# SunYangtian/Splatter_A_Video

Hardware: AMD Instinct MI355X
Metric: rendered frames/sec fwd+bwd @480p, 300k Gaussians (higher is better)
Workload: dtype f32

## Files before the change

splatter_a_video_amd/csrc/blend.hip:

```cpp
#include <stdlib.h>

#include <utility>

#include "common.h"
#include "blend_power.h"

struct BlendArgs {
    int P, C;
    int c0, cn;
    const float2 *uv;
    const float *conic;
    const float *opacity;
    const float *feature;
    const float *bias;
    const int *idx_sorted;
    const int2 *tile_range;
    float bg;
    const float *bgc;
    int W, H, gx;
    int K, trunc;
    float *out;
    float *final_T;
    int *ncontrib;
    int *gs_idx;
// ... 1033 lines not shown
    static constexpr int NA = (CH + 15) / 16;
    static constexpr int NK = (CH + 3) / 4;
    static constexpr bool SHARED = CH > 20;
    static constexpr int NSLAB = SHARED ? 1 : 4;
};

#define SCAN4(op, sh)                                                     \
    op " %0, %0, %0 row_shr:" sh " row_mask:0xf bank_mask:0xf\n\t"        \
    op " %1, %1, %1 row_shr:" sh " row_mask:0xf bank_mask:0xf\n\t"        \
    op " %2, %2, %2 row_shr:" sh " row_mask:0xf bank_mask:0xf\n\t"        \
    op " %3, %3, %3 row_shr:" sh " row_mask:0xf bank_mask:0xf\n\t"
__device__ __forceinline__ void row_scan_mul4(float &a, float &b, float &c, float &d) {
    asm volatile("s_nop 1\n\t" SCAN4("v_mul_f32_dpp", "1") SCAN4("v_mul_f32_dpp", "2") SCAN4("v_mul_f32_dpp", "4")
                     SCAN4("v_mul_f32_dpp", "8")
                 : "+v"(a), "+v"(b), "+v"(c), "+v"(d));
}
__device__ __forceinline__ void row_scan_add4(float &a, float &b, float &c, float &d) {
    asm volatile("s_nop 1\n\t" SCAN4("v_add_f32_dpp", "1") SCAN4("v_add_f32_dpp", "2") SCAN4("v_add_f32_dpp", "4")
                     SCAN4("v_add_f32_dpp", "8")
                 : "+v"(a), "+v"(b), "+v"(c), "+v"(d));
}
__device__ __forceinline__ void lds_store2_lane15(float *p, float a, float b) {
    const unsigned addr = (unsigned)(size_t)p;
    asm volatile(
        "s_mov_b64 exec, %3\n\t"
        "ds_write2_b32 %0, %1, %2 offset1:1\n\t"
        "s_mov_b64 exec, -1"
        :
        : "v"(addr), "v"(a), "v"(b), "s"(0x8000800080008000ull)
        : "memory");
}

template <int O0, int O1, int O2, int O3>
__device__ __forceinline__ void lds_store2x4_lane15(float *base, float a0, float b0, float a1, float b1, float a2, float b2, float a3,
                                                    float b3) {
    static_assert(O0 >= 0 && O1 >= 0 && O2 >= 0 && O3 >= 0 && O0 < 255 && O1 < 255 && O2 < 255 && O3 < 255, "ds_write2_b32 offsets are 8-bit dword counts");
    const unsigned addr = (unsigned)(size_t)base;
    asm volatile(
        "s_mov_b64 exec, %9\n\t"
        "ds_write2_b32 %0, %1, %2 offset0:%c10 offset1:%c11\n\t"
        "ds_write2_b32 %0, %3, %4 offset0:%c12 offset1:%c13\n\t"
        "ds_write2_b32 %0, %5, %6 offset0:%c14 offset1:%c15\n\t"
        "ds_write2_b32 %0, %7, %8 offset0:%c16 offset1:%c17\n\t"
        "s_mov_b64 exec, -1"
        :
        : "v"(addr), "v"(a0), "v"(b0), "v"(a1), "v"(b1), "v"(a2), "v"(b2), "v"(a3), "v"(b3), "s"(0x8000800080008000ull), "n"(O0),
          "n"(O0 + 1), "n"(O1), "n"(O1 + 1), "n"(O2), "n"(O2 + 1), "n"(O3), "n"(O3 + 1)
        : "memory");
}

typedef unsigned u32x2_b __attribute__((ext_vector_type(2)));
__device__ __forceinline__ float rows_sum(float v, int lane) {
    (void)lane;
    {
        const u32x2_b r = __builtin_amdgcn_permlane16_swap(__float_as_uint(v), __float_as_uint(v), false, false);
        v = __uint_as_float(r[0]) + __uint_as_float(r[1]);
    }
    {
        const u32x2_b r = __builtin_amdgcn_permlane32_swap(__float_as_uint(v), __float_as_uint(v), false, false);
        v = __uint_as_float(r[0]) + __uint_as_float(r[1]);
    }
    return v;
}

__device__ __forceinline__ void row_shr1_add4(float (&R)[4], const float (&rs)[4], const float (&base)[4]) {
    asm volatile(
        "s_nop 1\n\t"
        "v_add_f32_dpp %0, %4, %8 row_shr:1 row_mask:0xf bank_mask:0xf bound_ctrl:1\n\t"
        "v_add_f32_dpp %1, %5, %9 row_shr:1 row_mask:0xf bank_mask:0xf bound_ctrl:1\n\t"
        "v_add_f32_dpp %2, %6, %10 row_shr:1 row_mask:0xf bank_mask:0xf bound_ctrl:1\n\t"
        "v_add_f32_dpp %3, %7, %11 row_shr:1 row_mask:0xf bank_mask:0xf bound_ctrl:1\n\t"
        : "=&v"(R[0]), "=&v"(R[1]), "=&v"(R[2]), "=&v"(R[3])
        : "v"(rs[0]), "v"(rs[1]), "v"(rs[2]), "v"(rs[3]), "v"(base[0]), "v"(base[1]), "v"(base[2]), "v"(base[3]));
}


template <int QP>
struct QuarterWalk {
    static constexpr float CEN = 0.5f * (float)(QP + 3);
    static __device__ __forceinline__ int qx(int q) { return QP * ((q >> 4) & 1) + (q & 3); }
    static __device__ __forceinline__ int qy(int q) { return QP * (q >> 5) + ((q >> 2) & 3); }
};

template <typename Walk>
__device__ __forceinline__ void strip_phi(int nl, int kk, float ox, float oy, float (&phi1)[4], float (&phi2)[4]) {
#pragma unroll
    for (int Gs = 0; Gs < 4; ++Gs) {
        const int q = 16 * Gs + nl;
        const float x = (float)Walk::qx(q) + ox, y = (float)Walk::qy(q) + oy;
        phi1[Gs] = kk == 0 ? 1.f : kk == 1 ? x : kk == 2 ? y : x * x;
        phi2[Gs] = kk == 0 ? x * y : kk == 1 ? y * y : 0.f;
    }
}

template <typename Walk>
__device__ __forceinline__ void strip_moment_table(float (&s_mom)[16 * 32], int w, int nl, int kk) {
#pragma unroll
    for (int r = 0; r < 4; ++r) {
        const int st = 4 * w + r, Gs = st >> 2, is = st & 3;
        const int q = 16 * Gs + 4 * kk + is;
        const float x = (float)Walk::qx(q) - Walk::CEN, y = (float)Walk::qy(q) - Walk::CEN;
        float v = 0.f;
        if (nl < 4) v = nl == 0 ? 1.f : nl == 1 ? x : nl == 2 ? y : x * x;
        else if (nl < 6) v = nl == 4 ? x * y : y * y;
        if (nl < 8) s_mom[32 * st + 8 * kk + nl] = v;
    }
}

template <int SB>
__device__ __forceinline__ unsigned load_flags(const unsigned int *cull_flags, int tid, int first, int topb) {
    const int q = topb - tid;
    return (tid < SB && q >= 0) ? (unsigned)cull_flags[first + q] : 0u;
}

template <int SB, bool TRANSPOSE, int NKEEP>
__device__ __forceinline__ void keep_from_quarter_flags(unsigned int (&s_keep)[NKEEP], const int (&s_wmax)[4], int tid, int nb, int top, unsigned fl) {
    static_assert(NKEEP >= SB, "a keep word per staged entry");
    if (tid < SB) {
        unsigned kw = 0u;
        if (tid < nb) {
#pragma unroll
            for (int ww = 0; ww < 4; ++ww) {
                if (TRANSPOSE) {
                    const unsigned t4 = (fl >> ww) & 0x01010101u;
                    const unsigned nib = ((t4 * 0x01020408u) >> 24) & 0xfu;
                    if (top - tid < s_wmax[ww]) kw |= nib << (8 * ww);
                } else {
                    if (top - tid < s_wmax[ww]) kw |= fl & (0xfu << (8 * ww));
                }
            }
        }
        s_keep[tid] = kw;
    }
}

__device__ __forceinline__ unsigned wave_scan_bytes4(unsigned word) {
    unsigned incl = word;
    asm volatile("s_nop 1\n\t"
                 "v_add_u32_dpp %0, %0, %0 row_shr:1 row_mask:0xf bank_mask:0xf\n\t"
                 "s_nop 1\n\t"
                 "v_add_u32_dpp %0, %0, %0 row_shr:2 row_mask:0xf bank_mask:0xf\n\t"
                 "s_nop 1\n\t"
                 "v_add_u32_dpp %0, %0, %0 row_shr:4 row_mask:0xf bank_mask:0xf\n\t"
                 "s_nop 1\n\t"
                 "v_add_u32_dpp %0, %0, %0 row_shr:8 row_mask:0xf bank_mask:0xf\n\t"
                 "s_nop 1\n\t"
                 "v_add_u32_dpp %0, %0, %0 row_bcast:15 row_mask:0xa bank_mask:0xf\n\t"
                 "s_nop 1\n\t"
                 "v_add_u32_dpp %0, %0, %0 row_bcast:31 row_mask:0xc bank_mask:0xf\n\t"
                 : "+v"(incl));
    return incl;
}

template <int SB, int CAP, int RW, bool ROUNDS, int NKEEP, typename List>
__device__ __forceinline__ int build_quarter_lists(const unsigned int (&s_keep)[NKEEP], unsigned int (&s_pos4)[NKEEP], List list, float *slab,
                                                   int w, int lane, int (&cq)[4], int p0 = 0, int *more = nullptr) {
    static_assert(ROUNDS || CAP >= SB, "one round: a slab row per staged entry");
    static_assert(NKEEP >= (SB + WAVE - 1) / WAVE * WAVE, "every lane of a pass reads a keep word");
    unsigned cqw = 0u;
    int cnt = 0;
#pragma unroll
    for (int r = 0; r < (SB + WAVE - 1) / WAVE; ++r) {
        const int e = r * WAVE + lane;
        unsigned bits = (s_keep[e] >> (8 * w)) & 0xfu;
        const bool kb = bits != 0u;
        const unsigned long long m = __builtin_amdgcn_ballot_w64(kb);
        const int ps = cnt + __builtin_amdgcn_mbcnt_hi((unsigned)(m >> 32), __builtin_amdgcn_mbcnt_lo((unsigned)m, 0u));
        if (!ROUNDS) reinterpret_cast<unsigned char *>(s_pos4)[4 * e + w] = kb ? (unsigned char)ps : (unsigned char)255;
        else if (p0 == 0) reinterpret_cast<unsigned char *>(s_pos4)[4 * e + w] = kb ? (unsigned char)imin_(ps, 254) : (unsigned char)255;
        if (ROUNDS) bits = ((unsigned)(ps - p0) < (unsigned)CAP) ? bits : 0u;
        const unsigned word = (bits * 0x00204081u) & 0x01010101u;
        const unsigned incl = wave_scan_bytes4(word);
        const unsigned posw = cqw + incl - word;
        const unsigned short ent = (unsigned short)(e | ((ROUNDS ? ps - p0 : ps) << 8));
#pragma unroll
        for (int q = 0; q < 4; ++q)
            if ((bits >> q) & 1u) list(q, (posw >> (8 * q)) & 0xffu) = ent;
        cqw += (unsigned)__builtin_amdgcn_readlane((int)incl, 63);
        cnt += __popcll(m);
    }
#pragma unroll
    for (int q = 0; q < 4; ++q) cq[q] = (int)((cqw >> (8 * q)) & 0xffu);
    if (lane < 16) {
#pragma unroll
        for (int q = 0; q < 4; ++q) list(q, cq[q] + lane) = (unsigned short)(SB | (CAP << 8));
    }
    {
        const int rows = ROUNDS ? imin_(imax_(cnt - p0, 0), CAP) : cnt;
        float4 *z = reinterpret_cast<float4 *>(slab);
        for (int c = lane; c < rows * (RW / 4); c += WAVE) z[c] = make_float4(0.f, 0.f, 0.f, 0.f);
    }
    if (ROUNDS && lane == 0) *more = cnt > p0 + CAP;
    __builtin_amdgcn_fence(__ATOMIC_RELEASE, "wavefront");
    __builtin_amdgcn_wave_barrier();
    return cnt;
}

template <int NSEC, int LAST, int RS>
struct QuadStager {
    int id_next;
    float4 v[NSEC];

    __device__ __forceinline__ QuadStager() {
        if (LAST < 4) v[NSEC - 1] = make_float4(0.f, 0.f, 0.f, 0.f);
    }
    template <typename Pos>
    __device__ __forceinline__ void load_ids(const BlendArgs &A, int tid, int base, Pos pos, int batch) {
        const int q = pos(tid >> 2, batch);
        id_next = q >= 0 ? A.idx_sorted[base + q] : -1;
    }
    __device__ __forceinline__ void load_payload(const BlendArgs &A, int tid) {
        const int sp = tid & 3;
        const float4 *src = reinterpret_cast<const float4 *>(A.pack + (size_t)imax_(id_next, 0) * RS) + sp;
#pragma unroll
        for (int k = 0; k < NSEC - 1; ++k) v[k] = src[4 * k];
        if (LAST == 4 || (LAST > 0 && sp < LAST)) v[NSEC - 1] = src[4 * (NSEC - 1)];
    }
};

__device__ __forceinline__ void pair_exchange_geometry(const float4 &mine, bool first, float4 &g0, float4 &g1) {
    float4 other;
    other.x = __int_as_float(__builtin_amdgcn_mov_dpp(__float_as_int(mine.x), 0xB1, 0xf, 0xf, true));
    other.y = __int_as_float(__builtin_amdgcn_mov_dpp(__float_as_int(mine.y), 0xB1, 0xf, 0xf, true));
    other.z = __int_as_float(__builtin_amdgcn_mov_dpp(__float_as_int(mine.z), 0xB1, 0xf, 0xf, true));
    other.w = __int_as_float(__builtin_amdgcn_mov_dpp(__float_as_int(mine.w), 0xB1, 0xf, 0xf, true));
    g0 = first ? mine : other;
    g1 = first ? other : mine;
}

__device__ __forceinline__ void store_T_front(const BlendArgs &A, int px, int py, const float &t) {
    if (A.dbg_T_front) {
        if (px < A.W && py < A.H) A.dbg_T_front[(size_t)A.W * py + px] = t;
    }
}

template <int CH, int NK, int NA>
__device__ __forceinline__ void hoist_dl_dout(float *stage, const float (&gpix)[CH], int lane, float (&hcg)[4][NK], float (&hft)[16][NA]) {
    const int nl = lane & 15, kk = lane >> 4;
#pragma unroll
    for (int h = 0; h < 2; ++h) {
        if ((lane >> 5) == h) {
#pragma unroll
            for (int k = 0; k < CH; ++k) stage[(lane & 31) * CH + k] = gpix[k];
        }
        __builtin_amdgcn_fence(__ATOMIC_RELEASE, "wavefront");
        __builtin_amdgcn_wave_barrier();
#pragma unroll
        for (int G = 2 * h; G < 2 * h + 2; ++G)
#pragma unroll
            for (int j = 0; j < NK; ++j) hcg[G][j] = stage[(16 * (G & 1) + nl) * CH + 4 * j + kk];
#pragma unroll
        for (int st = 8 * h; st < 8 * h + 8; ++st) {
#pragma unroll
            for (int q = 0; q < NA; ++q)
                hft[st][q] = 16 * q + nl < CH ? stage[(16 * ((st >> 2) & 1) + 4 * kk + (st & 3)) * CH + 16 * q + nl] : 0.f;
        }
        __builtin_amdgcn_fence(__ATOMIC_ACQUIRE, "wavefront");
        __builtin_amdgcn_wave_barrier();
    }
}

template <int CH, bool ABS, bool EXACT>
__global__ void __launch_bounds__(256, (MfmaCfg<CH, ABS>::MINW))
blend_bwd_mfma_kernel(const BlendArgs B) {
    using Cfg = MfmaCfg<CH, ABS>;
    constexpr int SB = Cfg::SB, NG = Cfg::NG, NC = Cfg::NC, NCP = Cfg::NCP, PW = Cfg::PW, NA = Cfg::NA, NK = Cfg::NK;
    constexpr int PZ = Cfg::PZ, PS = Cfg::PS;
    constexpr int I_ABS = GradLayout<ABS, false>::I_ABS;
    constexpr bool SHARED = Cfg::SHARED;
    constexpr bool CARRY = CH <= 20;
    constexpr int CQ = CarryLDS<SB>::CQ, XR = CARRY ? 4 * CQ : 0;
    constexpr int CAP = SHARED ? (1 << 20) : (!CARRY ? SB : ((SB == 128 && NC <= 9) ? 80 : 64));
    constexpr int TPR = (NC + 2) / 3, NCS = SHARED ? 3 * TPR : NC;
    constexpr int SROWS = SHARED ? SB + XR : CAP + (CARRY ? 1 : 0);
    __shared__ TileLDS<CH, SB, false, XR, true> L;
    __shared__ CarryLDS<SB, !SHARED> CL;
    constexpr bool FEAT_VALU = CH <= 4;
    __shared__ float s_acc[Cfg::NSLAB][SROWS * NCS];
    constexpr int KS = 4 * PW + 8, GS = 4 * KS;
    __shared__ __attribute__((aligned(16))) float s_pix[4][4 * GS];
    auto pixoff = [](int q) { return (q >> 4) * GS + ((q >> 2) & 3) * KS + (q & 3) * PW; };
    __shared__ float s_mom[16 * 64];
    __shared__ int s_wmax[4];
    const int tid = threadIdx.x, lane = tid & 63, w = tid >> 6;
    const int gtile = xcd_tile(blockIdx.x, gridDim.x);
    const int frame = gtile / B.T, tile = gtile - frame * B.T;
    const BlendArgs A = frame_args(B, frame);
    const int RST = B.rec_stride ? B.rec_stride : NCP;
    float *const pair_buf = B.pair_buf + (size_t)frame * (size_t)B.cap * RST + B.rec_off;
    const int tx = tile % A.gx, ty = tile / A.gx;
    const int bx = tx * TILE + (w & 1) * 8, by = ty * TILE + (w >> 1) * 8;
    const float bx0 = (float)bx, by0 = (float)by;
    const float tcx = (float)(tx * TILE) + 7.5f, tcy = (float)(ty * TILE) + 7.5f;
    const float ox = (float)((w & 1) * 8) - 7.5f, oy = (float)((w >> 1) * 8) - 7.5f;
    const int cn = EXACT ? CH : A.cn;
    const int nl = lane & 15, kk = lane >> 4;
    int wmax;
#pragma unroll
    for (int r = 0; r < 4; ++r) {
        const int st = 4 * w + r, Gs = st >> 2, is = st & 3;
        const int q = 16 * Gs + 4 * kk + is;
        const float x = (float)(q & 7) - 3.5f, y = (float)(q >> 3) - 3.5f;
        const int grp = nl >> 2, i = nl & 3;
        float v = 0.f;
        if (grp == 0) v = i == 0 ? 1.f : i == 1 ? x : i == 2 ? y : x * x;
        if (grp == 1) v = i == 0 ? 1.f : i == 1 ? x : i == 2 ? y : x * y;
        if (grp == 2) v = i == 0 ? 1.f : i == 1 ? y : i == 2 ? y * y : 0.f;
        s_mom[64 * st + lane] = v;
    }
    float phi1[4], phi2[4];
#pragma unroll
    for (int Gs = 0; Gs < 4; ++Gs) {
        const int q = 16 * Gs + nl;
        const float x = (float)(q & 7) + ox, y = (float)(q >> 3) + oy;
        phi1[Gs] = kk == 0 ? 1.f : kk == 1 ? x : kk == 2 ? y : x * x;
        phi2[Gs] = kk == 0 ? x * y : kk == 1 ? y * y : 0.f;
    }
    {
        const int px = bx + (lane & 7), py = by + (lane >> 3);
        const size_t HW = (size_t)A.H * A.W;
        const bool inside = (px < A.W) && (py < A.H);
        const size_t pix = (size_t)A.W * (size_t)py + px;
        const float Tf = inside ? A.final_T[pix] : 0.f;
        const int last = inside ? A.ncontrib[pix] : 0;
        float *r = s_pix[w] + pixoff(lane);
        float bgdot = 0.f;
#pragma unroll
        for (int k = 0; k < CH; ++k) {
            const float g = (inside && k < cn) ? A.dL_dout[(size_t)(A.c0 + k) * HW + pix] : 0.f;
            r[k] = g;
            bgdot += A.bg * g;
        }
#pragma unroll
        for (int k = CH; k < PS; ++k) r[k] = 0.f;
        r[PS] = 0.f;
        r[PS + 1] = __int_as_float(last);
        r[PS + 2] = Tf;
        r[PS + 3] = Tf * bgdot;
// ... 209 lines not shown
            }
            if (j0 + nl < nproc) {
                float *rec = slab + (SHARED ? (e > SB ? e - 1 : e) : (CARRY ? j0 + nl - p0 : e)) * NCS;
                auto put = [](float *p, float v) {
                    if (SHARED) __hip_atomic_fetch_add(p, v, __ATOMIC_RELAXED, __HIP_MEMORY_SCOPE_WORKGROUP);
                    else *p = v;
                };
                const float D0 = d_mom[0];
                if (kk == 0) {
                    const float Dx = d_mom[1], Dy = d_mom[2], Dxx = d_mom[3];
                    put(rec + 0, cA * Dx + cB * Dy - (cA * uc + cB * vc) * D0);
                    put(rec + 1, cB * Dx + cC * Dy - (cB * uc + cC * vc) * D0);
                    put(rec + 2, -0.5f * (uc * uc * D0 - 2.f * uc * Dx + Dxx));
                    put(rec + 5, o > 0.f ? D0 / o : 0.f);
                    if (ABS) {
                        put(rec + I_ABS, s_ax);
                        put(rec + I_ABS + 1, s_ay);
                    }
                } else if (kk == 1) {
                    const float Dx = d_mom[1], Dy = d_mom[2], Dxy = d_mom[3];
                    put(rec + 3, -(uc * vc * D0 - uc * Dy - vc * Dx + Dxy));
                } else if (kk == 2) {
                    const float Dy = d_mom[1], Dyy = d_mom[2];
                    put(rec + 4, -0.5f * (vc * vc * D0 - 2.f * vc * Dy + Dyy));
                }
                if (FEAT_VALU) {
                    if (kk == 3) {
#pragma unroll
                        for (int c = 0; c < (FEAT_VALU ? CH : 1); ++c) put(rec + NG + c, dfv[c]);
                    }
                } else {
#pragma unroll
                    for (int q = 0; q < NA; ++q)
#pragma unroll
                        for (int i = 0; i < 4; ++i) {
                            const int c = 16 * q + 4 * kk + i;
                            if (c < CH) put(rec + NG + c, d_f[q][i]);
                        }
                }
            }
        }
        if (CARRY && p0 == 0) {
            __builtin_amdgcn_fence(__ATOMIC_RELEASE, "wavefront");
            __builtin_amdgcn_wave_barrier();
            if (nproc > 0)
                for (int idx = lane; idx < ncin * NC; idx += 64) {
                    const int k = idx / NC, c = idx - k * NC;
                    float *src = SHARED ? slab + (SB + CQ * w + k) * NCS + c : slab + idx;
                    __hip_atomic_fetch_add(pair_buf + (size_t)CL.cslot[w][k] * RST + c, *src, __ATOMIC_RELAXED,
                                           __HIP_MEMORY_SCOPE_AGENT);
                    if (SHARED) *src = 0.f;
                }
            const int left = total - nproc;
            if (left > 0) carry_out<CH, SB>(L, CL, w, lane, nproc > 0 ? nproc : ncin, nproc > 0 ? left : left - ncin,
                                            nproc > 0 ? 0 : ncin, top, slots);
            ncarry = left;
        }
        if (CARRY && !SHARED && lane == 0) CL.more[w] = nproc > p0 + CAP;
        if (p0 == 0) {
            load_slots();
            st.load_payload(A, tid);
            st.load_ids(A, tid, range.x, pos, batch + 2);
        }
        __syncthreads();
        if (ce < EPI) {
            const int lo = top - nb + 1;
            if (SHARED) {
#pragma unroll
                for (int r = 0; r < NPASS; ++r) {
                    const int ql = ce + r * EPI;
                    if (ql < nb) {
                        float *row = s_acc[0] + (nb - 1 - ql) * NCS + CW * cc;
                        const float v0 = row[0], v1 = row[CW > 1 ? 1 : 0], v2 = row[CW > 1 ? 2 : 0];
                        row[0] = 0.f;
                        if (CW > 1) { row[1] = 0.f; row[2] = 0.f; }
                        store_part(NPASS <= 3 ? sl[NPASS <= 3 ? r : 0] : slots[lo + ql], v0, v1, v2);
                    }
                }
            } else {
#pragma unroll
                for (int r = 0; r < NPASS; ++r) {
                    const int ql = ce + r * EPI;
                    if (ql < nb) {
                        const unsigned int p4 = CL.pos4[nb - 1 - ql];
                        float v[3] = {0.f, 0.f, 0.f};
#pragma unroll
                        for (int ww = 0; ww < 4; ++ww) {
                            const unsigned int pp = umin_(((p4 >> (8 * ww)) & 0xffu) - (unsigned)p0, (unsigned)CAP);
                            const float *row = s_acc[ww] + pp * NC + CW * cc;
#pragma unroll
                            for (int j = 0; j < 3; ++j)
                                if (CW * (TPR - 1) + j < NC || CW * cc + j < NC) v[j] += row[j];
                        }
                        const int slot = NPASS <= 3 ? sl[NPASS <= 3 ? r : 0] : slots[lo + ql];
                        if (p0 > 0) {
                            const float *old = pair_buf + (size_t)slot * RST + CW * cc;
#pragma unroll
                            for (int j = 0; j < 3; ++j)
                                if (CW * cc + j < NCP) v[j] += old[j];
                        }
                        store_part(slot, v[0], v[1], v[2]);
                    }
                }
            }
        }
        if (SHARED) break;
        const bool more = CARRY && (CL.more[0] | CL.more[1] | CL.more[2] | CL.more[3]);
        __syncthreads();
        if (!more) break;
        }
    }
    if (A.dbg_T_front) {
        const int px = bx + (lane & 7), py = by + (lane >> 3);
        if (px < A.W && py < A.H) A.dbg_T_front[(size_t)A.W * py + px] = s_pix[w][pixoff(lane) + PS + 2];
    }
}

#define ROW_LANES(X) X(0) X(1) X(2) X(3) X(4) X(5) X(6) X(7) X(8) X(9) X(10) X(11) X(12) X(13) X(14) X(15)
__device__ __forceinline__ void fmac_row_lane(int n, float &acc, float src, float w) {
    switch (n) {
#define ROW_CASE(N) case N: asm("v_fmac_f32_dpp %0, %1, %2 row_newbcast:" #N " row_mask:0xf bank_mask:0xf" : "+v"(acc) : "v"(src), "v"(w)); break;
        ROW_LANES(ROW_CASE)
#undef ROW_CASE
    }
}
__device__ __forceinline__ void mul_row_lane(int n, float &acc, float src, float w) {
    switch (n) {
#define ROW_CASE(N) case N: asm("v_mul_f32_dpp %0, %1, %2 row_newbcast:" #N " row_mask:0xf bank_mask:0xf" : "=&v"(acc) : "v"(src), "v"(w)); break;
        ROW_LANES(ROW_CASE)
#undef ROW_CASE
    }
}
__device__ __forceinline__ int row_lane(int n, int v) {
    switch (n) {
#define ROW_CASE(N) case N: return __builtin_amdgcn_update_dpp(0, v, 0x150 + N, 0xf, 0xf, true);
        ROW_LANES(ROW_CASE)
#undef ROW_CASE
    }
    return v;
}
#undef ROW_LANES

template <int CH, bool ABS = false>
struct QuarterCfg {
    static_assert(CH <= 3 && Rec<CH>::RQ == 4 && Rec<CH>::CULL >= 11, "floats 11-15 of the record (cull parameters) are free for the coefficients");
    static constexpr int SB = 128;
    static constexpr int CAP = 80;
    static constexpr int MINW = ABS ? 3 : 4;
    static constexpr int NG = GradLayout<ABS, false>::NG, NC = NG + CH, NCP = PAIR_STRIDE(NC);
    static constexpr int RW = ABS ? 16 : 12;
    static constexpr int PW = 8;
};

template <int CH, bool ABS, bool EXACT>
__global__ void __launch_bounds__(256, (QuarterCfg<CH, ABS>::MINW))
blend_bwd_quarter_kernel(const BlendArgs B) {
    using Cfg = QuarterCfg<CH, ABS>;
    constexpr int SB = Cfg::SB, CAP = Cfg::CAP, NCP = Cfg::NCP, RW = Cfg::RW, PW = Cfg::PW, RQ = 4;
    static_assert(SB <= 128 && CAP < 255, "list entries are (entry | position << 8) in 16 bits");
    __shared__ float4 s_rec[(SB + 1) * RQ];
    auto qpart = [](int e, int p) { return 4 * e + (p ^ ((e >> 2) & 3)); };
    __shared__ unsigned int s_keep[SB];
    __shared__ unsigned short s_qlist[4][4][CAP + 16];
    __shared__ unsigned int s_pos4[SB];
    __shared__ __attribute__((aligned(16))) float s_acc[4][(CAP + 1) * RW];
    constexpr int KS = 4 * PW + 8, GS = 4 * KS;
    __shared__ __attribute__((aligned(16))) float s_pix[4][4 * GS];
    auto pixoff = [](int q) { return (q >> 4) * GS + ((q >> 2) & 3) * KS + (q & 3) * PW; };
    __shared__ float s_mom[16 * 32];
    __shared__ int s_wmax[4];
    __shared__ int s_more[4];
    const int tid = threadIdx.x, lane = tid & 63, w = tid >> 6;
    const int gtile = xcd_tile(blockIdx.x, gridDim.x);
    const int frame = gtile / B.T, tile = gtile - frame * B.T;
    const BlendArgs A = frame_args(B, frame);
    const int RST = B.rec_stride ? B.rec_stride : NCP;
    float *const pair_buf = B.pair_buf + (size_t)frame * (size_t)B.cap * RST + B.rec_off;
    const int tx = tile % A.gx, ty = tile / A.gx;
    const int bx = tx * TILE + (w & 1) * 8, by = ty * TILE + (w >> 1) * 8;
    const float tcx = (float)(tx * TILE) + 7.5f, tcy = (float)(ty * TILE) + 7.5f;
    const float ox = (float)((w & 1) * 8) - 7.5f, oy = (float)((w >> 1) * 8) - 7.5f;
    const int cn = EXACT ? CH : A.cn;
    const int nl = lane & 15, kk = lane >> 4;
    using Walk = QuarterWalk<4>;
#pragma unroll
    for (int r = 0; r < 4; ++r) {
        const int st = 4 * w + r, Gs = st >> 2, is = st & 3;
        const int q = 16 * Gs + 4 * kk + is;
        const float x = (float)Walk::qx(q) - Walk::CEN, y = (float)Walk::qy(q) - Walk::CEN;
        float v = 0.f;
        if (ABS) {
            if (nl < 4) v = nl == 0 ? 1.f : nl == 1 ? x : nl == 2 ? y : x * x;
            else if (nl < 6) v = nl == 4 ? x * y : y * y;
        } else {
            if (nl < 3) v = nl == 0 ? 1.f : nl == 1 ? x : y;
            else if (nl >= 4 && nl < 7) v = nl == 4 ? x * x : nl == 5 ? x * y : y * y;
        }
        if (nl < 8) s_mom[32 * st + 8 * kk + nl] = v;
    }
    float phi1[4], phi2[4];
    strip_phi<Walk>(nl, kk, ox, oy, phi1, phi2);
    const int lx = lane & 7, ly = lane >> 3;
    const int myq = 16 * ((lx >> 2) + 2 * (ly >> 2)) + 4 * (ly & 3) + (lx & 3);
    {
        const int px = bx + lx, py = by + ly;
        const size_t HW = (size_t)A.H * A.W;
        const bool inside = (px < A.W) && (py < A.H);
        const size_t pix = (size_t)A.W * (size_t)py + px;
        const float Tf = inside ? A.final_T[pix] : 0.f;
        const int last = inside ? A.ncontrib[pix] : 0;
        float *r = s_pix[w] + pixoff(myq);
        float bgdot = 0.f;
#pragma unroll
        for (int k = 0; k < 4; ++k) {
            const float g = (k < CH && inside && k < cn) ? A.dL_dout[(size_t)(A.c0 + k) * HW + pix] : 0.f;
            r[k] = g;
            bgdot += A.bg * g;
        }
        r[4] = 0.f;
        r[5] = __int_as_float(last);
        r[6] = Tf;
        r[7] = Tf * bgdot;
        const int wmax = wave_max_i(last);
        if (lane == 0) s_wmax[w] = wmax;
    }
    if (tid < RQ) s_rec[qpart(SB, tid)] = make_float4(tid == 3 ? -__builtin_inff() : 0.f, 0.f, 0.f, 0.f);
    if (lane < RW) s_acc[w][CAP * RW + lane] = 0.f;
    __syncthreads();
    const int2 range = A.tile_range[tile];
    const int len = range.y - range.x;
    const int n = imin_(len, imax_(imax_(s_wmax[0], s_wmax[1]), imax_(s_wmax[2], s_wmax[3])));
    const int *slots = A.slot_sorted + range.x;
    auto store_rec = [&](int slot, const float (&v)[12]) {
        float4 *dst = reinterpret_cast<float4 *>(pair_buf + (size_t)slot * RST);
#pragma unroll
        for (int c = 0; c < NCP / 4; ++c) dst[c] = make_float4(v[4 * c], v[4 * c + 1], v[4 * c + 2], v[4 * c + 3]);
    };
    {
        const float z[12] = {0.f, 0.f, 0.f, 0.f, 0.f, 0.f, 0.f, 0.f, 0.f, 0.f, 0.f, 0.f};
        for (int ql = n + tid; ql < len; ql += 256) store_rec(slots[ql], z);
    }
    if (n <= 0) {
        store_T_front(A, bx + lx, by + ly, s_pix[w][pixoff(myq) + 6]);
        return;
    }
    float *pixrow = s_pix[w] + kk * KS;
    float gpix[3];
    int lastpix;
    {
        const float *r = s_pix[w] + (nl >> 2) * GS + kk * KS + (nl & 3) * PW;
        gpix[0] = r[0]; gpix[1] = r[1]; gpix[2] = r[2];
        lastpix = __float_as_int(r[5]);
    }
    const float *pixcol = s_pix[w] + pixoff(nl);
    const float *momrow = s_mom + 8 * kk + (nl & 7);
    const int kch = kk < CH ? kk : 4;

    auto pos = [n](int e, int b) { return n - 1 - b * SB - e; };
    Stager<CH, SB> st;
    static_assert(Stager<CH, SB>::NCHUNK % 256 == 0, "every thread parks K chunks");
    st.load_ids(A, tid, range.x, pos, 0);
    st.load_payload(A, tid);
    st.load_ids(A, tid, range.x, pos, 1);
    unsigned fl_next = load_flags<SB>(A.cull_flags, tid, range.x, n - 1);

    int batch = 0;
    for (int top = n - 1; top >= 0; top -= SB, ++batch) {
        const int nb = imin_(SB, top + 1);
        {
            const int p = tid & 3;
#pragma unroll
            for (int k = 0; k < Stager<CH, SB>::K; ++k) {
                const int e = (tid >> 2) + 64 * k;
                const float4 mine = st.v[k];
                float4 g0, g1;
                pair_exchange_geometry(mine, p == 0, g0, g1);
                const PowerCoef pc = power_coeffs(g0.x, g0.y, g0.z, g0.w, g1.x, g1.y, tcx, tcy);
                if (p == 0) {
                    s_rec[qpart(e, 0)] = mine;
                    s_rec[qpart(e, 3)] = make_float4(pc.q0, pc.qx, pc.qy, pc.qxx);
                } else if (p == 1) {
                    s_rec[qpart(e, 1)] = make_float4(mine.x, mine.y, pc.qxy, pc.qyy);
                } else if (p == 2) {
                    s_rec[qpart(e, 2)] = make_float4(mine.x, mine.y, mine.z, 0.f);
                }
            }
        }
        const unsigned fl = fl_next;
        fl_next = load_flags<SB>(A.cull_flags, tid, range.x, top - SB);
        keep_from_quarter_flags<SB, false>(s_keep, s_wmax, tid, nb, top, fl);
        __syncthreads();
        float *slab = s_acc[w];
        int slot_mine = 0;
        for (int p0 = 0;; p0 += CAP) {
            int cq[4];
            build_quarter_lists<SB, CAP, RW, true>(s_keep, s_pos4, [&](int q, int i) -> unsigned short & { return s_qlist[w][q][i]; }, slab, w, lane, cq, p0,
                                                   &s_more[w]);
#pragma unroll
            for (int G = 0; G < 4; ++G) {
                const float cgA = pixcol[G * GS + kch];
                float momA[4];
#pragma unroll
                for (int i = 0; i < 4; ++i) momA[i] = momrow[32 * (4 * G + i)];
                for (int j0 = 0; j0 < cq[G]; j0 += 16) {
                    const unsigned le = s_qlist[w][G][j0 + nl];
                    const int e = le & 0xffu, row = le >> 8;
                    const int qn = top - e;
                    const float *er = reinterpret_cast<const float *>(s_rec) + e * (4 * RQ);
                    const int sw = 4 * ((e >> 2) & 3);
                    const float bq1 = er[(12 ^ sw) + kk];
                    const float bq2 = er[(4 ^ sw) + 2 + (kk & 1)];
                    const float bf = er[(8 ^ sw) + kk];
                    float blx = 0.f, bly = 0.f;
                    if (ABS) {
                        const float4 ge = *reinterpret_cast<const float4 *>(er + (0 ^ sw));
                        const float cCe = er[(4 ^ sw)];
                        const float ut = ge.x - tcx, vt = ge.y - tcy;
                        blx = kk == 0 ? -(ge.z * ut + ge.w * vt) : kk == 1 ? ge.z : kk == 2 ? ge.w : 0.f;
                        bly = kk == 0 ? -(ge.w * ut + cCe * vt) : kk == 1 ? ge.w : kk == 2 ? cCe : 0.f;
                    }
                    float s_ax = 0.f, s_ay = 0.f;
                    f32x4 d_mom = {0.f, 0.f, 0.f, 0.f};
                    float dfv[CH];
                    asm volatile("" ::: "memory");
                    f32x4 pw = {0.f, 0.f, 0.f, 0.f}, cgv = {0.f, 0.f, 0.f, 0.f};
                    pw = __builtin_amdgcn_mfma_f32_16x16x4f32(phi1[G], bq1, pw, 0, 0, 0);
                    pw = __builtin_amdgcn_mfma_f32_16x16x4f32(phi2[G], bq2, pw, 0, 0, 0);
                    cgv = __builtin_amdgcn_mfma_f32_16x16x4f32(cgA, bf, cgv, 0, 0, 0);
                    float cg[4], araw[4], a[4], r1a[4], rp[4], Ts4[4], Rs4[4];
#pragma unroll
                    for (int i = 0; i < 4; ++i) {
                        const float2 stv = *reinterpret_cast<const float2 *>(pixrow + G * GS + i * PW + 6);
                        cg[i] = cgv[i];
                        const int last = row_lane(4 * G + i, lastpix);
                        Ts4[i] = stv.x;
                        Rs4[i] = stv.y;
                        bool pw_ok;
                        araw[i] = exp2_guard(pw[i], pw_ok);
                        const bool ok = (qn < last) && pw_ok && !(araw[i] < (1.0f / 255.0f));
                        araw[i] = ok ? araw[i] : 0.f;
                        a[i] = fminf(0.99f, araw[i]);
                        r1a[i] = __builtin_amdgcn_rcpf(1.f - a[i]);
                        rp[i] = r1a[i];
                    }
                    row_scan_mul4(rp[0], rp[1], rp[2], rp[3]);
                    float T[4], wgt[4], rs[4], R[4];
#pragma unroll
                    for (int i = 0; i < 4; ++i) {
                        T[i] = Ts4[i] * rp[i];
                        wgt[i] = a[i] * T[i];
                        rs[i] = cg[i] * wgt[i];
                    }
                    row_scan_add4(rs[0], rs[1], rs[2], rs[3]);
                    row_shr1_add4(R, rs, Rs4);
                    lds_store2x4_lane15<6, PW + 6, 2 * PW + 6, 3 * PW + 6>(pixrow + G * GS, T[0], Rs4[0] + rs[0], T[1], Rs4[1] + rs[1], T[2],
                                                                           Rs4[2] + rs[2], T[3], Rs4[3] + rs[3]);
                    f32x4 lx4 = {0.f, 0.f, 0.f, 0.f}, ly4 = {0.f, 0.f, 0.f, 0.f};
                    if (ABS) {
                        lx4 = __builtin_amdgcn_mfma_f32_16x16x4f32(phi1[G], blx, lx4, 0, 0, 0);
                        ly4 = __builtin_amdgcn_mfma_f32_16x16x4f32(phi1[G], bly, ly4, 0, 0, 0);
                    }
#pragma unroll
                    for (int i = 0; i < 4; ++i) {
                        const float dLa = T[i] * cg[i] - R[i] * r1a[i];
                        const float dLp = araw[i] * dLa;
                        d_mom = __builtin_amdgcn_mfma_f32_16x16x4f32(momA[i], dLp, d_mom, 0, 0, 0);
                        if (ABS) {
                            s_ax += fabsf(dLp * lx4[i]);
                            s_ay += fabsf(dLp * ly4[i]);
                        }
#pragma unroll
                        for (int c = 0; c < CH; ++c) {
                            if (i == 0) mul_row_lane(4 * G, dfv[c], gpix[c], wgt[0]);
                            else fmac_row_lane(4 * G + i, dfv[c], gpix[c], wgt[i]);
                        }
                    }
                    if (ABS) {
                        s_ax = rows_sum(s_ax, lane);
                        s_ay = rows_sum(s_ay, lane);
                    }
                    float fs[3] = {0.f, 0.f, 0.f};
#pragma unroll
                    for (int c = 0; c < CH; ++c) {
                        const u32x2_b r = __builtin_amdgcn_permlane32_swap(__float_as_uint(dfv[c]), __float_as_uint(dfv[c]), false, false);
                        fs[c] = __uint_as_float(r[0]) + __uint_as_float(r[1]);
                    }
                    if (!ABS) {
                        if (j0 + nl < cq[G]) {
                            F3 *r3 = reinterpret_cast<F3 *>(slab + row * RW + 3 * kk);
                            F3 v3 = *r3;
                            v3.x += kk < 2 ? d_mom[0] : fs[0];
                            v3.y += kk < 2 ? d_mom[1] : fs[1];
                            v3.z += kk < 2 ? d_mom[2] : fs[2];
                            *r3 = v3;
                        }
                    } else if (kk < 2 && j0 + nl < cq[G]) {
                        float4 *rm = reinterpret_cast<float4 *>(slab + row * RW + 4 * kk), *rf = rm + 2;
                        float4 m4 = *rm, f4 = *rf;
                        m4.x += d_mom[0]; m4.y += d_mom[1];
                        m4.z += ABS ? d_mom[2] + (kk == 1 ? s_ax : 0.f) : d_mom[2];
                        m4.w += ABS ? d_mom[3] + (kk == 1 ? s_ay : 0.f) : d_mom[3];
                        f4.x += fs[0]; f4.y += fs[1]; f4.z += fs[2];
                        *rm = m4;
                        *rf = f4;
                    }
                    __builtin_amdgcn_fence(__ATOMIC_RELEASE, "wavefront");
                    __builtin_amdgcn_wave_barrier();
                }
            }
            if (p0 == 0) {
                slot_mine = tid < nb ? slots[top - tid] : 0;
                st.load_payload(A, tid);
                st.load_ids(A, tid, range.x, pos, batch + 2);
            }
            __syncthreads();
            if (tid < nb) {
                const int e = tid;
                const unsigned int p4 = s_pos4[e];
                float s[12] = {0.f, 0.f, 0.f, 0.f, 0.f, 0.f, 0.f, 0.f, 0.f, 0.f, 0.f, 0.f};
#pragma unroll
                for (int ww = 0; ww < 4; ++ww) {
                    const unsigned int pp = umin_(((p4 >> (8 * ww)) & 0xffu) - (unsigned)p0, (unsigned)CAP);
                    const float4 *rw = reinterpret_cast<const float4 *>(s_acc[ww] + pp * RW);
                    float4 m, m2, fa, fb;
                    if (ABS) {
                        m = rw[0]; m2 = rw[1]; fa = rw[2]; fb = rw[3];
                    } else {
                        const float4 r1 = rw[1], r2 = rw[2];
                        m = rw[0];
                        m2 = make_float4(r1.x, r1.y, 0.f, 0.f);
                        fa = make_float4(r1.z, r1.w, r2.x, 0.f);
                        fb = make_float4(r2.y, r2.z, r2.w, 0.f);
                    }
                    const float bxw = (ww & 1) ? 4.f : -4.f, byw = (ww >> 1) ? 4.f : -4.f;
                    s[0] += m.x;
                    s[1] += m.y + bxw * m.x;
                    s[2] += m.z + byw * m.x;
                    s[3] += m.w + 2.f * bxw * m.y + (bxw * bxw) * m.x;
                    s[4] += m2.x + bxw * m.z + byw * m.y + (bxw * byw) * m.x;
                    s[5] += m2.y + 2.f * byw * m.z + (byw * byw) * m.x;
                    s[6] += fa.x + fb.x; s[7] += fa.y + fb.y; s[8] += fa.z + fb.z;
                    s[9] += m2.z; s[10] += m2.w;
                }
                const float4 g0 = s_rec[qpart(e, 0)], g1 = s_rec[qpart(e, 1)];
                const float cA = g0.z, cB = g0.w, cC = g1.x, o = g1.y;
                const float uc = g0.x - tcx, vc = g0.y - tcy;
                const float M0 = s[0], Mx = s[1], My = s[2], Mxx = s[3], Mxy = s[4], Myy = s[5];
                float rec[12];
                rec[0] = cA * Mx + cB * My - (cA * uc + cB * vc) * M0;
                rec[1] = cB * Mx + cC * My - (cB * uc + cC * vc) * M0;
                rec[2] = -0.5f * (uc * uc * M0 - 2.f * uc * Mx + Mxx);
                rec[3] = -(uc * vc * M0 - uc * My - vc * Mx + Mxy);
                rec[4] = -0.5f * (vc * vc * M0 - 2.f * vc * My + Myy);
                rec[5] = o > 0.f ? M0 / o : 0.f;
                rec[6] = 0.f; rec[7] = 0.f; rec[8] = 0.f; rec[9] = 0.f; rec[10] = 0.f; rec[11] = 0.f;
                if (ABS) { rec[6] = s[9]; rec[7] = s[10]; }
                rec[Cfg::NG] = s[6];
                if (CH > 1) rec[Cfg::NG + 1 % CH] = s[7];
                if (CH > 2) rec[Cfg::NG + 2 % CH] = s[8];
                if (p0 > 0) {
                    const float *old = pair_buf + (size_t)slot_mine * RST;
#pragma unroll
                    for (int c = 0; c < Cfg::NC; ++c) rec[c] += old[c];
                }
                store_rec(slot_mine, rec);
            }
            const bool more = s_more[0] | s_more[1] | s_more[2] | s_more[3];
            __syncthreads();
            if (!more) break;
        }
    }
    store_T_front(A, bx + lx, by + ly, s_pix[w][pixoff(myq) + 6]);
}

struct SetsCfg {
    static constexpr int CH = 28, NK = 7, NA = 2, SB = 64;
    static constexpr int NG = SETS_NG, NCMAX = NG + CH;
    static constexpr int PS = 8;
    static constexpr int MINW = 2;
    static constexpr int CAP = 32;
};

__device__ __forceinline__ constexpr int sets_fpos(int slot) { return 8 + 8 * (slot & 3) + (slot >> 2); }

__device__ __forceinline__ int sets_slot_channel(const BlendArgs &A, int slot) {
    const int g = slot < 4 ? 0 : slot < 8 ? 1 : 2;
    const int o = slot - (g == 0 ? 0 : g == 1 ? 4 : 8);
    const int c0 = g == 0 ? A.s0c0 : g == 1 ? A.s1c0 : A.s2c0, cn = g == 0 ? A.s0cn : g == 1 ? A.s1cn : A.s2cn;
    return (slot < SetsCfg::CH && o < cn) ? c0 + o : -1;
}

__global__ void __launch_bounds__(256)
pack_sets_kernel(const BlendArgs B) {
    const BlendArgs A = frame_args(B, blockIdx.y);
    constexpr int CH = SetsCfg::CH, RS = Rec<CH>::RS, CO = Rec<CH>::CULL;
    static_assert(CO >= 0, "the cull parameters ride in the record's padding");
    constexpr int RQ = Rec<CH>::RQ, LS = RS + 4;
    __shared__ __attribute__((aligned(16))) float s_rec[256 * LS];
    const int i0 = blockIdx.x * 256;
    const int i = i0 + threadIdx.x;
    float r[RS];
#pragma unroll
    for (int k = 0; k < RS; ++k) r[k] = 0.f;
    if (i < A.P) {
        const float2 q = A.uv[i];
        r[0] = q.x; r[1] = q.y;
        r[2] = A.conic[3 * i]; r[3] = A.conic[3 * i + 1]; r[4] = A.conic[3 * i + 2];
        r[5] = A.opacity[i];
        r[7] = __int_as_float(i);
        if (A.feature) {
            const float *f = A.feature + (size_t)i * (A.feature_row ? A.feature_row : A.C);
#pragma unroll
            for (int k = 0; k < CH; ++k) {
                const int c = sets_slot_channel(A, k);
                if (c >= 0) r[sets_fpos(k)] = f[c];
            }
        }
        const CullP cp = cull_params(r[2], r[3], r[4], r[5]);
        r[CO] = cp.hx; r[CO + 1] = cp.hy; r[CO + 2] = cp.tauq; r[CO + 3] = cp.ia; r[CO + 4] = cp.ic;
    }
    float4 *row = reinterpret_cast<float4 *>(s_rec + threadIdx.x * LS);
#pragma unroll
    for (int k = 0; k < RS; k += 4) row[k / 4] = make_float4(r[k], r[k + 1], r[k + 2], r[k + 3]);
    __syncthreads();
    const int nrec = imin_(256, A.P - i0);
    if (!A.feature) {
        stage_feature_rows<true>(s_rec, LS, 0, A.sf0, A.s0cn, i0, nrec);
        stage_feature_rows<true>(s_rec, LS, 4, A.sf1, A.s1cn, i0, nrec);
        stage_feature_rows<true>(s_rec, LS, 8, A.sf2, A.s2cn, i0, nrec);
        __syncthreads();
    }
    float4 *dst = reinterpret_cast<float4 *>(A.pack + (size_t)i0 * RS);
    for (int c = threadIdx.x; c < nrec * RQ; c += 256) {
        const int g = c / RQ, part = c - g * RQ;
        dst[c] = *reinterpret_cast<const float4 *>(s_rec + g * LS + 4 * part);
    }
}

template <bool ABS>
__global__ void __launch_bounds__(256, SetsCfg::MINW)
blend_bwd_sets_kernel(const BlendArgs B) {
    using Cfg = SetsCfg;
    constexpr int CH = Cfg::CH, SB = Cfg::SB, NG = Cfg::NG, NK = Cfg::NK, NA = Cfg::NA, PS = Cfg::PS;
    constexpr int CAP = Cfg::CAP;
    static_assert(CAP % 16 == 0 && (CAP + 1) * Cfg::NCMAX >= 32 * CH, "whole chunks; the staging of 32 pixels fits a slab");
    __shared__ TileLDS<CH, SB, false, 0, true> L;
    __shared__ CarryLDS<SB, true> CL;
    __shared__ float s_acc[4][(CAP + 1) * Cfg::NCMAX];
    constexpr int KS = 4 * PS + 8, GS = 4 * KS;
    __shared__ __attribute__((aligned(16))) float s_state[4][4 * GS];
    auto pixoff = [](int q) { return (q >> 4) * GS + ((q >> 2) & 3) * KS + (q & 3) * PS; };
    __shared__ float s_mom[16 * 64];
    __shared__ int s_wmax[4];
    const int tid = threadIdx.x, lane = tid & 63, w = tid >> 6;
    const int gtile = xcd_tile(blockIdx.x, gridDim.x);
    const int frame = gtile / B.T, tile = gtile - frame * B.T;
    const BlendArgs A = frame_args(B, frame);
    const int NC = NG + A.C, NCP = PAIR_STRIDE(NC);
    float *const pair_buf = B.pair_buf + (size_t)frame * (size_t)B.cap * NCP;
    const int tx = tile % A.gx, ty = tile / A.gx;
// ... 1931 lines not shown
```

Measured before the change: 5593.

## Add lean backward blend path skipping per-pixel contributor checks when batch is fully below

```diff
diff --git a/splatter_a_video_amd/csrc/blend.hip b/splatter_a_video_amd/csrc/blend.hip
--- a/splatter_a_video_amd/csrc/blend.hip
+++ b/splatter_a_video_amd/csrc/blend.hip
@@ -1209,11 +1209,12 @@
     return incl;
 }
 
-template <int SB, int CAP, int RW, bool ROUNDS, int NKEEP, typename List>
+template <int SB, int CAP, int RW, bool ROUNDS, int PAD = CAP, int NKEEP, typename List>
 __device__ __forceinline__ int build_quarter_lists(const unsigned int (&s_keep)[NKEEP], unsigned int (&s_pos4)[NKEEP], List list, float *slab,
                                                    int w, int lane, int (&cq)[4], int p0 = 0, int *more = nullptr) {
     static_assert(ROUNDS || CAP >= SB, "one round: a slab row per staged entry");
     static_assert(NKEEP >= (SB + WAVE - 1) / WAVE * WAVE, "every lane of a pass reads a keep word");
+    static_assert(PAD >= CAP && PAD < 256, "the pad row lies behind the rows of a round, its number in the entry's high byte");
     unsigned cqw = 0u;
     int cnt = 0;
 #pragma unroll
@@ -1240,7 +1241,7 @@
     for (int q = 0; q < 4; ++q) cq[q] = (int)((cqw >> (8 * q)) & 0xffu);
     if (lane < 16) {
 #pragma unroll
-        for (int q = 0; q < 4; ++q) list(q, cq[q] + lane) = (unsigned short)(SB | (CAP << 8));
+        for (int q = 0; q < 4; ++q) list(q, cq[q] + lane) = (unsigned short)(SB | (PAD << 8));
     }
     {
         const int rows = ROUNDS ? imin_(imax_(cnt - p0, 0), CAP) : cnt;
@@ -1756,18 +1757,25 @@
     static constexpr int PW = 8;
 };
 
+template <bool V>
+struct BoolC { static constexpr bool value = V; };
+typedef float __attribute__((address_space(3))) lds_float;
+typedef f32x4 __attribute__((address_space(3))) lds_f32x4;
+#define LDS_F32(addr) (reinterpret_cast<const lds_float *>((size_t)(addr)))
+#define LDS_F32X4(addr) (reinterpret_cast<const lds_f32x4 *>((size_t)(addr)))
+
 template <int CH, bool ABS, bool EXACT>
 __global__ void __launch_bounds__(256, (QuarterCfg<CH, ABS>::MINW))
 blend_bwd_quarter_kernel(const BlendArgs B) {
     using Cfg = QuarterCfg<CH, ABS>;
     constexpr int SB = Cfg::SB, CAP = Cfg::CAP, NCP = Cfg::NCP, RW = Cfg::RW, PW = Cfg::PW, RQ = 4;
-    static_assert(SB <= 128 && CAP < 255, "list entries are (entry | position << 8) in 16 bits");
-    __shared__ float4 s_rec[(SB + 1) * RQ];
+    static_assert(SB <= 128 && CAP + 1 < 255, "list entries are (entry | position << 8) in 16 bits");
+    __shared__ __attribute__((aligned(64))) float4 s_rec[(SB + 1) * RQ];
     auto qpart = [](int e, int p) { return 4 * e + (p ^ ((e >> 2) & 3)); };
     __shared__ unsigned int s_keep[SB];
     __shared__ unsigned short s_qlist[4][4][CAP + 16];
     __shared__ unsigned int s_pos4[SB];
-    __shared__ __attribute__((aligned(16))) float s_acc[4][(CAP + 1) * RW];
+    __shared__ __attribute__((aligned(16))) float s_acc[4][(CAP + 2) * RW];
     constexpr int KS = 4 * PW + 8, GS = 4 * KS;
     __shared__ __attribute__((aligned(16))) float s_pix[4][4 * GS];
     auto pixoff = [](int q) { return (q >> 4) * GS + ((q >> 2) & 3) * KS + (q & 3) * PW; };
@@ -1829,7 +1837,7 @@
         if (lane == 0) s_wmax[w] = wmax;
     }
     if (tid < RQ) s_rec[qpart(SB, tid)] = make_float4(tid == 3 ? -__builtin_inff() : 0.f, 0.f, 0.f, 0.f);
-    if (lane < RW) s_acc[w][CAP * RW + lane] = 0.f;
+    if (lane < 2 * RW) s_acc[w][CAP * RW + lane] = 0.f;
     __syncthreads();
     const int2 range = A.tile_range[tile];
     const int len = range.y - range.x;
@@ -1856,6 +1864,23 @@
         gpix[0] = r[0]; gpix[1] = r[1]; gpix[2] = r[2];
         lastpix = __float_as_int(r[5]);
     }
+    int lmin[4];
+    {
+        int m = lastpix;
+        m = imin_(m, __builtin_amdgcn_mov_dpp(m, 0xB1, 0xf, 0xf, true));
+        m = imin_(m, __builtin_amdgcn_mov_dpp(m, 0x4E, 0xf, 0xf, true));
+        {
+            const u32x2_b r = __builtin_amdgcn_permlane16_swap((unsigned)m, (unsigned)m, false, false);
+            m = imin_((int)r[0], (int)r[1]);
+        }
+        {
+            const u32x2_b r = __builtin_amdgcn_permlane32_swap((unsigned)m, (unsigned)m, false, false);
+            m = imin_((int)r[0], (int)r[1]);
+        }
+#pragma unroll
+        for (int G = 0; G < 4; ++G) lmin[G] = __builtin_amdgcn_readlane(m, 4 * G);
+    }
+    const unsigned recbase = (unsigned)(size_t)s_rec + 48u + 4u * (unsigned)kk;
     const float *pixcol = s_pix[w] + pixoff(nl);
     const float *momrow = s_mom + 8 * kk + (nl & 7);
     const int kch = kk < CH ? kk : 4;
@@ -1898,27 +1923,24 @@
         int slot_mine = 0;
         for (int p0 = 0;; p0 += CAP) {
             int cq[4];
-            build_quarter_lists<SB, CAP, RW, true>(s_keep, s_pos4, [&](int q, int i) -> unsigned short & { return s_qlist[w][q][i]; }, slab, w, lane, cq, p0,
-                                                   &s_more[w]);
-#pragma unroll
-            for (int G = 0; G < 4; ++G) {
-                const float cgA = pixcol[G * GS + kch];
-                float momA[4];
-#pragma unroll
-                for (int i = 0; i < 4; ++i) momA[i] = momrow[32 * (4 * G + i)];
-                for (int j0 = 0; j0 < cq[G]; j0 += 16) {
+            build_quarter_lists<SB, CAP, RW, true, CAP + 1>(s_keep, s_pos4, [&](int q, int i) -> unsigned short & { return s_qlist[w][q][i]; }, slab, w, lane,
+                                                            cq, p0, &s_more[w]);
+            auto step = [&](auto lean_c, const int G, const int j0, const float cgA, const float (&momA)[4]) __attribute__((always_inline)) {
+                    constexpr bool LEAN = decltype(lean_c)::value;
                     const unsigned le = s_qlist[w][G][j0 + nl];
                     const int e = le & 0xffu, row = le >> 8;
                     const int qn = top - e;
-                    const float *er = reinterpret_cast<const float *>(s_rec) + e * (4 * RQ);
-                    const int sw = 4 * ((e >> 2) & 3);
-                    const float bq1 = er[(12 ^ sw) + kk];
-                    const float bq2 = er[(4 ^ sw) + 2 + (kk & 1)];
-                    const float bf = er[(8 ^ sw) + kk];
+                    unsigned a3 = recbase + ((unsigned)e << 6);
+                    asm("" : "+v"(a3));
+                    a3 ^= (le & 0xcu) << 2;
+                    const float bq1 = *LDS_F32(a3);
+                    const float bq2 = LDS_F32((a3 & ~8u) ^ 32u)[2];
+                    const float bf = *LDS_F32(a3 ^ 16u);
                     float blx = 0.f, bly = 0.f;
                     if (ABS) {
-                        const float4 ge = *reinterpret_cast<const float4 *>(er + (0 ^ sw));
-                        const float cCe = er[(4 ^ sw)];
+                        const f32x4 gv = *LDS_F32X4((a3 & ~12u) ^ 48u);
+                        const float4 ge = make_float4(gv[0], gv[1], gv[2], gv[3]);
+                        const float cCe = *LDS_F32((a3 & ~12u) ^ 32u);
                         const float ut = ge.x - tcx, vt = ge.y - tcy;
                         blx = kk == 0 ? -(ge.z * ut + ge.w * vt) : kk == 1 ? ge.z : kk == 2 ? ge.w : 0.f;
                         bly = kk == 0 ? -(ge.w * ut + cCe * vt) : kk == 1 ? ge.w : kk == 2 ? cCe : 0.f;
@@ -1936,12 +1958,12 @@
                     for (int i = 0; i < 4; ++i) {
                         const float2 stv = *reinterpret_cast<const float2 *>(pixrow + G * GS + i * PW + 6);
                         cg[i] = cgv[i];
-                        const int last = row_lane(4 * G + i, lastpix);
                         Ts4[i] = stv.x;
                         Rs4[i] = stv.y;
                         bool pw_ok;
                         araw[i] = exp2_guard(pw[i], pw_ok);
-                        const bool ok = (qn < last) && pw_ok && !(araw[i] < (1.0f / 255.0f));
+                        bool ok = pw_ok && !(araw[i] < (1.0f / 255.0f));
+                        if (!LEAN) ok = (qn < row_lane(4 * G + i, lastpix)) && ok;
                         araw[i] = ok ? araw[i] : 0.f;
                         a[i] = fminf(0.99f, araw[i]);
                         r1a[i] = __builtin_amdgcn_rcpf(1.f - a[i]);
@@ -1990,7 +2012,7 @@
                         fs[c] = __uint_as_float(r[0]) + __uint_as_float(r[1]);
                     }
                     if (!ABS) {
-                        if (j0 + nl < cq[G]) {
+                        {
                             F3 *r3 = reinterpret_cast<F3 *>(slab + row * RW + 3 * kk);
                             F3 v3 = *r3;
                             v3.x += kk < 2 ? d_mom[0] : fs[0];
@@ -1998,7 +2020,7 @@
                             v3.z += kk < 2 ? d_mom[2] : fs[2];
                             *r3 = v3;
                         }
-                    } else if (kk < 2 && j0 + nl < cq[G]) {
+                    } else if (kk < 2) {
                         float4 *rm = reinterpret_cast<float4 *>(slab + row * RW + 4 * kk), *rf = rm + 2;
                         float4 m4 = *rm, f4 = *rf;
                         m4.x += d_mom[0]; m4.y += d_mom[1];
@@ -2010,6 +2032,17 @@
                     }
                     __builtin_amdgcn_fence(__ATOMIC_RELEASE, "wavefront");
                     __builtin_amdgcn_wave_barrier();
+            };
+#pragma unroll
+            for (int G = 0; G < 4; ++G) {
+                const float cgA = pixcol[G * GS + kch];
+                float momA[4];
+#pragma unroll
+                for (int i = 0; i < 4; ++i) momA[i] = momrow[32 * (4 * G + i)];
+                if (top < lmin[G]) {
+                    for (int j0 = 0; j0 < cq[G]; j0 += 16) step(BoolC<true>{}, G, j0, cgA, momA);
+                } else {
+                    for (int j0 = 0; j0 < cq[G]; j0 += 16) step(BoolC<false>{}, G, j0, cgA, momA);
                 }
             }
             if (p0 == 0) {
```

After: 5647, median of 6. No clear change (+1.0%).
